# barathanaslan/whisper-ipa

Hardware: AMD Instinct MI355X
Metric: audio-seconds/sec transcribed (whisper-small, 30s clips) (higher is better)
Workload: dtype bf16

## Files before the change

### whisper_ipa_amd/csrc/attention.hip

```cpp
#include <cstring>

#include "attn_stream.h"
#include "wipa_common.h"

namespace {

struct AttnParams {
    const char* q;
    const char* k;
    const char* v;
    char* out;
    const int32_t* tk_dev;
    const int32_t* q_row_dev;
    float* lse;
    int64_t q_bs, q_rs, q_hs, k_bs, k_rs, k_hs, v_bs, v_rs, v_hs, o_bs, o_rs, o_hs;
    int Tq, Tk, causal, H;
};

template <bool RAGGED, bool GROUPED = false>
struct AttnArgs : AttnParams {};
template <>
struct AttnArgs<true> : AttnParams {
    const int32_t* k_start;
};
// ... 313 lines not shown
        Vec16<T> qv = *reinterpret_cast<const Vec16<T>*>(qp);
#pragma unroll
        for (int e = 0; e < EPL; ++e) qf[t][e] = qv.get(e);
    }
    int kvb = b;
    if constexpr (GROUPED) kvb = b / p.n_group;
    const T* Kb = reinterpret_cast<const T*>(p.k) + kvb * p.k_bs + h * p.k_hs + c * EPL;
    const T* Vb = reinterpret_cast<const T*>(p.v) + kvb * p.v_bs + h * p.v_hs + c * EPL;
    const int64_t k_rs = p.k_rs, v_rs = p.v_rs;
    float m[NQ], l[NQ], acc[NQ][EPL];
#pragma unroll
    for (int t = 0; t < NQ; ++t) {
        m[t] = NEG_BIG;
        l[t] = 0.f;
#pragma unroll
        for (int e = 0; e < EPL; ++e) acc[t][e] = 0.f;
    }
    constexpr int STEP = 4 * G * U;
    for (int t0 = wave * G * U; t0 < Tk; t0 += STEP) {
        Vec16<T> ka[U], va[U];
#pragma unroll
        for (int u = 0; u < U; ++u) {
            ka[u] = load_row_clamped(Kb, t0 + u * G + g, Tk - 1, k_rs);
            va[u] = load_row_clamped(Vb, t0 + u * G + g, Tk - 1, v_rs);
        }
#pragma unroll
        for (int t = 0; t < NQ; ++t) WIPA_STREAM_STEP(U, qf[t], ka, va, t0, m[t], l[t], acc[t]);
    }
#pragma unroll
    for (int t = 0; t < NQ; ++t) {
        WIPA_LANE_MERGE(LPK, 64, EPL, m[t], l[t], acc[t]);
        WIPA_WAVE_MERGE_STORE(s_acc[t], s_m[t], s_l[t], m[t], l[t], acc[t]);
    }
    __syncthreads();
    if (tid < 64 * NQ) {
        const int t = tid >> 6, dd = tid & 63;
        WIPA_WAVE_MERGE_OUT(s_acc[t], s_m[t], s_l[t], dd, reinterpret_cast<T*>(p.out)[b * p.o_bs + (int64_t)t * p.o_rs + h * p.o_hs + dd]);
    }
}

constexpr int FA_ROWB = 128;
constexpr int FA_TILE = 64 * FA_ROWB;
constexpr float LOG2E = 1.4426950408889634f;

#define WIPA_FLASH_SOFTMAX_TILE()                                                                  \
    do {                                                                                           \
        if (kt * 64 + 64 > T) {                                                                    \
            asm volatile("" ::: "memory");                                                         \
            _Pragma("unroll") for (int u = 0; u < 2; ++u)                                          \
                _Pragma("unroll") for (int i = 0; i < 16; ++i) {                                   \
                    const int key = kt * 64 + 32 * u + (i & 3) + 8 * (i >> 2) + 4 * hh;            \
                    if (key >= T) S[u][i] = NEG_BIG;                                               \
                }                                                                                  \
        }                                                                                          \
        float mx = NEG_BIG;                                                                        \
        _Pragma("unroll") for (int u = 0; u < 2; ++u)                                              \
            _Pragma("unroll") for (int i = 0; i < 16; ++i) mx = fmaxf(mx, S[u][i]);                \
        mx = fmaxf(mx, __shfl_xor(mx, 32, 64));                                                    \
        const float m_new = fmaxf(m, mx * LOG2E);                                                  \
        f32x2 psum2 = {0.f, 0.f};                                                                  \
        const f32x2 l2e = {LOG2E, LOG2E}, mneg = {-m_new, -m_new};                                 \
        _Pragma("unroll") for (int u = 0; u < 2; ++u)                                              \
            _Pragma("unroll") for (int i = 0; i < 16; i += 2) {                                    \
                const f32x2 x = __builtin_elementwise_fma(f32x2{S[u][i], S[u][i + 1]}, l2e, mneg); \
                const f32x2 pv = {__builtin_amdgcn_exp2f(x.x), __builtin_amdgcn_exp2f(x.y)};       \
                S[u][i] = pv.x;                                                                    \
                S[u][i + 1] = pv.y;                                                                \
                psum2 += pv;                                                                       \
            }                                                                                      \
        const float psum = psum2.x + psum2.y;                                                      \
        if (__any(m_new > m)) {                                                                    \
            const float alpha = __builtin_amdgcn_exp2f(m - m_new);                                 \
            l *= alpha;                                                                            \
            _Pragma("unroll") for (int i = 0; i < 16; ++i) {                                       \
                O[0][i] *= alpha;                                                                  \
                O[1][i] *= alpha;                                                                  \
            }                                                                                      \
            m = m_new;                                                                             \
        }                                                                                          \
        l += psum;                                                                                 \
    } while (0)
#define WIPA_FLASH_SOFTMAX_FINISH() l += __shfl_xor(l, 32, 64)

__global__ __launch_bounds__(512) void flash_enc_bf16_kernel(const __bf16* __restrict__ qk, int64_t ldqk,
                                                             const __bf16* __restrict__ vt, int64_t ldvt,
                                                             __bf16* __restrict__ out, int64_t ldo, int H, int T) {
    __shared__ __attribute__((aligned(16))) char smem[4 * FA_TILE];
    const int tid = threadIdx.x, lane = tid & 63, wave = tid >> 6;
    const int r = lane & 31, hh = lane >> 5;
    const int h = blockIdx.y, b = blockIdx.z;
    const int D = H * 64;
    const int nw = blockDim.x >> 6;
    const int q0 = blockIdx.x * (nw * 32) + wave * 32;
    const int nkt = (T + 63) / 64;

    bf16x8 qf[4];
    {
        const int qrow = min(q0 + r, T - 1);
        const __bf16* qp = qk + ((int64_t)b * T + qrow) * ldqk + h * 64 + 8 * hh;
#pragma unroll
        for (int s = 0; s < 4; ++s) qf[s] = *reinterpret_cast<const bf16x8*>(qp + 16 * s);
    }
    typedef __attribute__((address_space(3))) void* lds_t;
    const __bf16* kbase = qk + (int64_t)b * T * ldqk + D + h * 64;
    const __bf16* vbase = vt + ((int64_t)b * D + h * 64) * ldvt;
    const __amdgpu_buffer_rsrc_t rK = __builtin_amdgcn_make_buffer_rsrc((void*)kbase, 0, (int)(((int64_t)(T - 1) * ldqk + 64) * 2), 0x00020000);
    const __amdgpu_buffer_rsrc_t rV = __builtin_amdgcn_make_buffer_rsrc((void*)vbase, 0, (int)(((int64_t)63 * ldvt + ldvt) * 2), 0x00020000);
    const int wv = __builtin_amdgcn_readfirstlane(wave);
    const int ppw = 8 / nw;
    int offK[2], offV[2];
#pragma unroll
    for (int i = 0; i < 2; ++i) {
        const int row = 8 * (ppw * wv + i) + (lane >> 3);
        const int c = (lane & 7) ^ ((row >> 1) & 7);
        offK[i] = row * (int)ldqk * 2 + c * 16;
        offV[i] = row * (int)ldvt * 2 + c * 16;
    }
    auto stage = [&](int kt, int buf) {
        char* base = smem + buf * 2 * FA_TILE + (ppw * wv) * 1024;
        const int k0 = kt * 64;
#pragma unroll
        for (int i = 0; i < 2; ++i) {
            if (i < ppw) {
                __builtin_amdgcn_raw_ptr_buffer_load_lds(rK, (lds_t)(base + i * 1024), 16, offK[i], k0 * (int)ldqk * 2, 0, 0);
                __builtin_amdgcn_raw_ptr_buffer_load_lds(rV, (lds_t)(base + FA_TILE + i * 1024), 16, offV[i], k0 * 2, 0, 0);
            }
        }
    };

    f32x16 O[2];
#pragma unroll
    for (int i = 0; i < 16; ++i) O[0][i] = O[1][i] = 0.f;
    float m = NEG_BIG, l = 0.f;
    const int rsw = (r >> 1) & 7;

    stage(0, 0);
    asm volatile("s_waitcnt vmcnt(0)" ::: "memory");
    __syncthreads();
    for (int kt = 0; kt < nkt; ++kt) {
        if (kt + 1 < nkt) stage(kt + 1, (kt + 1) & 1);
        const char* kbuf = smem + (kt & 1) * 2 * FA_TILE;
        const char* vbuf = kbuf + FA_TILE;
        f32x16 S[2];
#pragma unroll
        for (int u = 0; u < 2; ++u) {
#pragma unroll
            for (int i = 0; i < 16; ++i) S[u][i] = 0.f;
            const char* krow = kbuf + (32 * u + r) * FA_ROWB;
#pragma unroll
            for (int s = 0; s < 4; ++s) {
                const bf16x8 kf = *reinterpret_cast<const bf16x8*>(krow + (((2 * s + hh) ^ rsw) << 4));
                S[u] = __builtin_amdgcn_mfma_f32_32x32x16_bf16(kf, qf[s], S[u], 0, 0, 0);
            }
        }
        WIPA_FLASH_SOFTMAX_TILE();
#pragma unroll
        for (int u = 0; u < 2; ++u)
#pragma unroll
            for (int sp = 0; sp < 2; ++sp) {
                bf16x8 pb;
#pragma unroll
                for (int j = 0; j < 8; ++j) pb[j] = (__bf16)S[u][8 * sp + j];
#pragma unroll
                for (int dt = 0; dt < 2; ++dt) {
                    const char* vrow = vbuf + (32 * dt + r) * FA_ROWB + 8 * hh;
                    const int c0 = 4 * u + 2 * sp;
                    const bf16x4 lo = *reinterpret_cast<const bf16x4*>(vrow + ((c0 ^ rsw) << 4));
                    const bf16x4 hi = *reinterpret_cast<const bf16x4*>(vrow + (((c0 + 1) ^ rsw) << 4));
                    const bf16x8 vf = {lo[0], lo[1], lo[2], lo[3], hi[0], hi[1], hi[2], hi[3]};
                    O[dt] = __builtin_amdgcn_mfma_f32_32x32x16_bf16(vf, pb, O[dt], 0, 0, 0);
                    asm volatile("" ::: "memory");
                }
            }
        asm volatile("s_waitcnt vmcnt(0)" ::: "memory");
        __syncthreads();
    }
    WIPA_FLASH_SOFTMAX_FINISH();
    const int qrow = q0 + r;
    if (qrow < T) {
        const float inv = 1.f / l;
        __bf16* op = out + ((int64_t)b * T + qrow) * ldo + h * 64 + 4 * hh;
#pragma unroll
        for (int dt = 0; dt < 2; ++dt)
#pragma unroll
            for (int g4 = 0; g4 < 4; ++g4) {
                bf16x4 o = {(__bf16)(O[dt][4 * g4] * inv), (__bf16)(O[dt][4 * g4 + 1] * inv),
                            (__bf16)(O[dt][4 * g4 + 2] * inv), (__bf16)(O[dt][4 * g4 + 3] * inv)};
                *reinterpret_cast<bf16x4*>(op + 32 * dt + 8 * g4) = o;
            }
    }
}

constexpr int FF_LD = 68;
constexpr int FF_TILE = 64 * FF_LD;

__device__ __forceinline__ void stage_k_parity(float* krow, int kseg, const f32x4 (&rk)[4]) {
    float* kt = krow + 8 * kseg;
    *reinterpret_cast<f32x4*>(kt) = f32x4{rk[0][0], rk[0][2], rk[1][0], rk[1][2]};
    *reinterpret_cast<f32x4*>(kt + 4) = f32x4{rk[2][0], rk[2][2], rk[3][0], rk[3][2]};
    *reinterpret_cast<f32x4*>(kt + 32) = f32x4{rk[0][1], rk[0][3], rk[1][1], rk[1][3]};
    *reinterpret_cast<f32x4*>(kt + 36) = f32x4{rk[2][1], rk[2][3], rk[3][1], rk[3][3]};
}
__device__ __forceinline__ void stage_k_plain(float* krow, int kseg, const f32x4 (&rk)[4]) {
    float* kt = krow + 16 * kseg;
#pragma unroll
    for (int c = 0; c < 4; ++c) *reinterpret_cast<f32x4*>(kt + 4 * c) = rk[c];
}

#define WIPA_FLASH_F32_INDICES()                                                                                 \
    __shared__ __attribute__((aligned(16))) float smem[4 * FF_TILE];     \
    const int tid = threadIdx.x, lane = tid & 63, wave = tid >> 6;                                               \
    const int r = lane & 31, hh = lane >> 5;                                                                     \
    const int h = blockIdx.y, b = blockIdx.z;                                                                    \
    const int q0 = blockIdx.x * 128 + wave * 32;                                                                 \
    const int nkt = (T + 63) / 64

#define WIPA_FLASH_F32_STAGING(STAGE_K)                                                                          \
    const int krow = tid >> 2, kseg = tid & 3;                                                                   \
    const int vkey = tid & 63, vseg = tid >> 6;                                                                  \
    const float* kg = k + (int64_t)b * T * ldk + h * 64 + 16 * kseg;                                             \
    const float* vg = v + (int64_t)b * T * ldv + h * 64 + 16 * vseg;                                             \
    f32x4 rk[4], rv[4];                                                                                          \
    auto gload = [&](int kt) {                                                                                   \
        const float* kp = kg + (int64_t)min(kt * 64 + krow, T - 1) * ldk;                                        \
        const float* vp = vg + (int64_t)min(kt * 64 + vkey, T - 1) * ldv;                                        \
        _Pragma("unroll") for (int c = 0; c < 4; ++c) {                                                          \
            rk[c] = *reinterpret_cast<const f32x4*>(kp + 4 * c);                                                 \
            rv[c] = *reinterpret_cast<const f32x4*>(vp + 4 * c);                                                 \
        }                                                                                                        \
    };                                                                                                           \
    auto swrite = [&](int buf) {                                                                                 \
        STAGE_K(smem + buf * 2 * FF_TILE + krow * FF_LD, kseg, rk);                                              \
        float* vt = smem + buf * 2 * FF_TILE + FF_TILE + (16 * vseg) * FF_LD + vkey;            \
        _Pragma("unroll") for (int c = 0; c < 4; ++c)                                                            \
            _Pragma("unroll") for (int e = 0; e < 4; ++e) vt[(4 * c + e) * FF_LD] = rv[c][e];                    \
    };                                                                                                           \
    f32x16 O[2];                                                                                                 \
    _Pragma("unroll") for (int i = 0; i < 16; ++i) O[0][i] = O[1][i] = 0.f;                                      \
    float m = NEG_BIG, l = 0.f;                                                        \
    gload(0);                                                                                                    \
    swrite(0);                                                                                                   \
    __syncthreads()

#define WIPA_FLASH_F32_TILE_BEGIN()                                                                              \
    if (kt + 1 < nkt) gload(kt + 1);                                                                             \
    const float* kbuf = smem + (kt & 1) * 2 * FF_TILE;                                                           \
    const float* vbuf = kbuf + FF_TILE;                                                                          \
    f32x16 S[2]
#define WIPA_FLASH_F32_TILE_END()                                                                                \
    if (kt + 1 < nkt) swrite((kt + 1) & 1);                                                                      \
    __syncthreads()

#define WIPA_FLASH_F32_TAIL()                                                                                    \
    WIPA_FLASH_SOFTMAX_FINISH();                                                                                 \
    const int qrow = q0 + r;                                                                                     \
    if (qrow < T) {                                                                                              \
        const float inv = 1.f / l;                                                                               \
        float* op = out + ((int64_t)b * T + qrow) * ldo + h * 64 + 4 * hh;                                       \
// ... 33 lines not shown
#pragma unroll
        for (int u = 0; u < 2; ++u)
#pragma unroll
            for (int dt = 0; dt < 2; ++dt) {
                const float* vr = vbuf + (32 * dt + r) * FF_LD + 32 * u + 4 * hh;
#pragma unroll
                for (int g = 0; g < 4; ++g) {
                    const f32x4 vf = *reinterpret_cast<const f32x4*>(vr + 8 * g);
#pragma unroll
                    for (int e = 0; e < 4; ++e)
                        O[dt] = __builtin_amdgcn_mfma_f32_32x32x2f32(vf[e], S[u][4 * g + e], O[dt], 0, 0, 0);
                }
            }
        WIPA_FLASH_F32_TILE_END();
    }
    WIPA_FLASH_F32_TAIL();
}

__global__ __launch_bounds__(256, 2) void flash_enc_f32s_kernel(const float* __restrict__ q, int64_t ldq,
                                                                const float* __restrict__ k, int64_t ldk,
                                                                const float* __restrict__ v, int64_t ldv,
                                                                float* __restrict__ out, int64_t ldo, int T) {
    WIPA_FLASH_F32_INDICES();
    bf16x8 qh[4], qm[4], ql[4];
    {
        const float* qp = q + ((int64_t)b * T + min(q0 + r, T - 1)) * ldq + h * 64 + 8 * hh;
#pragma unroll
        for (int s = 0; s < 4; ++s)
            split_bf16x3(*reinterpret_cast<const f32x4*>(qp + 16 * s), *reinterpret_cast<const f32x4*>(qp + 16 * s + 4), qh[s], qm[s], ql[s]);
    }
    WIPA_FLASH_F32_STAGING(stage_k_plain);
    for (int kt = 0; kt < nkt; ++kt) {
        WIPA_FLASH_F32_TILE_BEGIN();
#pragma unroll
        for (int u = 0; u < 2; ++u) {
#pragma unroll
            for (int i = 0; i < 16; ++i) S[u][i] = 0.f;
            const float* kr = kbuf + (32 * u + r) * FF_LD + 8 * hh;
#pragma unroll
            for (int s = 0; s < 4; ++s) {
                bf16x8 kh, km, kl;
                split_bf16x3(*reinterpret_cast<const f32x4*>(kr + 16 * s), *reinterpret_cast<const f32x4*>(kr + 16 * s + 4), kh, km, kl);
                S[u] = __builtin_amdgcn_mfma_f32_32x32x16_bf16(kl, qh[s], S[u], 0, 0, 0);
                S[u] = __builtin_amdgcn_mfma_f32_32x32x16_bf16(km, qm[s], S[u], 0, 0, 0);
                S[u] = __builtin_amdgcn_mfma_f32_32x32x16_bf16(kh, ql[s], S[u], 0, 0, 0);
                S[u] = __builtin_amdgcn_mfma_f32_32x32x16_bf16(km, qh[s], S[u], 0, 0, 0);
                S[u] = __builtin_amdgcn_mfma_f32_32x32x16_bf16(kh, qm[s], S[u], 0, 0, 0);
                S[u] = __builtin_amdgcn_mfma_f32_32x32x16_bf16(kh, qh[s], S[u], 0, 0, 0);
            }
        }
        WIPA_FLASH_SOFTMAX_TILE();
#pragma unroll
        for (int u = 0; u < 2; ++u)
#pragma unroll
            for (int sp = 0; sp < 2; ++sp) {
                bf16x8 ph, pl;
                split_bf16x2(f32x4{S[u][8 * sp], S[u][8 * sp + 1], S[u][8 * sp + 2], S[u][8 * sp + 3]},
                             f32x4{S[u][8 * sp + 4], S[u][8 * sp + 5], S[u][8 * sp + 6], S[u][8 * sp + 7]}, ph, pl);
#pragma unroll
                for (int dt = 0; dt < 2; ++dt) {
                    const float* vr = vbuf + (32 * dt + r) * FF_LD + 32 * u + 16 * sp + 4 * hh;
                    bf16x8 vh, vl;
                    split_bf16x2(*reinterpret_cast<const f32x4*>(vr), *reinterpret_cast<const f32x4*>(vr + 8), vh, vl);
                    O[dt] = __builtin_amdgcn_mfma_f32_32x32x16_bf16(vh, pl, O[dt], 0, 0, 0);
                    O[dt] = __builtin_amdgcn_mfma_f32_32x32x16_bf16(vl, ph, O[dt], 0, 0, 0);
                    O[dt] = __builtin_amdgcn_mfma_f32_32x32x16_bf16(vh, ph, O[dt], 0, 0, 0);
                }
            }
        WIPA_FLASH_F32_TILE_END();
    }
    WIPA_FLASH_F32_TAIL();
}

#undef WIPA_FLASH_F32_INDICES
#undef WIPA_FLASH_F32_STAGING
#undef WIPA_FLASH_F32_TILE_BEGIN
#undef WIPA_FLASH_F32_TILE_END
#undef WIPA_FLASH_F32_TAIL
#undef WIPA_FLASH_SOFTMAX_TILE
#undef WIPA_FLASH_SOFTMAX_FINISH

}

static bool attn_strides_aligned(const wipa_attn_desc* d) {
    const int64_t al = d->dtype == WIPA_BF16 ? 8 : 4;
    return d->q_rs % al == 0 && d->k_rs % al == 0 && d->v_rs % al == 0 && d->q_hs % al == 0 && d->k_hs % al == 0 && d->v_hs % al == 0 &&
           d->q_bs % al == 0 && d->k_bs % al == 0 && d->v_bs % al == 0;
}

static void fill_attn_params(const wipa_attn_desc* d, AttnParams& p) {
    p.q = (const char*)d->q;
    p.k = (const char*)d->k;
    p.v = (const char*)d->v;
    p.out = (char*)d->out;
    p.tk_dev = d->tk_dev;
    p.q_row_dev = d->q_row_dev;
    p.lse = d->lse;
    p.q_bs = d->q_bs; p.q_rs = d->q_rs; p.q_hs = d->q_hs;
    p.k_bs = d->k_bs; p.k_rs = d->k_rs; p.k_hs = d->k_hs;
    p.v_bs = d->v_bs; p.v_rs = d->v_rs; p.v_hs = d->v_hs;
    p.o_bs = d->o_bs; p.o_rs = d->o_rs; p.o_hs = d->o_hs;
    p.Tq = d->Tq;
    p.Tk = d->Tk;
    p.causal = d->causal;
    p.H = d->H;
}

extern "C" int wipa_attention(const wipa_attn_desc* d, wipa_stream_t stream) { return wipa_attention_as(d, d ? d->Tq : 0, stream); }

int wipa_attention_as(const wipa_attn_desc* d, int path_tq, wipa_stream_t stream) {
    WIPA_REQUIRE(d && d->q && d->k && d->v && d->out, "wipa_attention: null pointer");
    WIPA_REQUIRE(d->B > 0 && d->H > 0 && d->Tq > 0, "wipa_attention: bad shape");
    WIPA_REQUIRE(d->dtype == WIPA_F32 || d->dtype == WIPA_BF16, "wipa_attention: bad dtype %d", d->dtype);
    WIPA_REQUIRE(attn_strides_aligned(d), "wipa_attention: strides must keep 16-byte alignment");
    AttnArgs<false> p;
    fill_attn_params(d, p);
    dim3 grid((d->Tq + 15) / 16, d->H, d->B);
    static const bool valu = [] { const char* e = getenv("WIPA_ATTN_FWD"); return e && !strcmp(e, "valu"); }();
    if (d->dtype == WIPA_F32 && !valu && path_tq >= 16 && !d->tk_dev && !d->q_row_dev && d->o_rs % 4 == 0 && d->o_hs % 4 == 0 &&
        d->o_bs % 4 == 0) {
        hipLaunchKernelGGL(attn_fwd_f32_mfma_kernel, dim3((d->Tq + 63) / 64, d->H, d->B), dim3(256), 0, (hipStream_t)stream, p);
        WIPA_LAUNCH_CHECK();
        return WIPA_OK;
    }
    if (d->dtype == WIPA_F32)
        hipLaunchKernelGGL((attn_generic_kernel<float>), grid, dim3(256), 0, (hipStream_t)stream, p);
    else
        hipLaunchKernelGGL((attn_generic_kernel<__bf16>), grid, dim3(256), 0, (hipStream_t)stream, p);
    WIPA_LAUNCH_CHECK();
    return WIPA_OK;
}

extern "C" int wipa_attention_ragged(const wipa_attn_desc* d, const int32_t* starts_dev, wipa_stream_t stream) {
    WIPA_REQUIRE(d && d->q && d->k && d->v && d->out && starts_dev, "wipa_attention_ragged: null pointer (starts_dev is required)");
    WIPA_REQUIRE(d->B > 0 && d->H > 0 && d->Tq > 0, "wipa_attention_ragged: bad shape");
    WIPA_REQUIRE(d->dtype == WIPA_F32 || d->dtype == WIPA_BF16, "wipa_attention_ragged: bad dtype %d", d->dtype);
    WIPA_REQUIRE(attn_strides_aligned(d), "wipa_attention_ragged: strides must keep 16-byte alignment");
    WIPA_REQUIRE(d->causal && d->Tq == d->Tk && !d->tk_dev && !d->q_row_dev && !d->lse,
                 "wipa_attention_ragged: causal self-attention with Tq == Tk (Tq=%d Tk=%d), no device-side offsets, no lse", d->Tq, d->Tk);
    AttnArgs<true> p;
    fill_attn_params(d, p);
    p.k_start = starts_dev;
    dim3 grid((d->Tq + 15) / 16, d->H, d->B);
    if (d->dtype == WIPA_F32)
        hipLaunchKernelGGL((attn_generic_kernel<float, true>), grid, dim3(256), 0, (hipStream_t)stream, p);
    else
        hipLaunchKernelGGL((attn_generic_kernel<__bf16, true>), grid, dim3(256), 0, (hipStream_t)stream, p);
    WIPA_LAUNCH_CHECK();
    return WIPA_OK;
}

extern "C" int wipa_flash_attn_enc_bf16(const void* qk, int64_t ldqk, const void* vt, int64_t ldvt, void* out, int64_t ldo,
                                        int B, int H, int T, wipa_stream_t stream) {
    WIPA_REQUIRE(qk && vt && out, "wipa_flash_attn_enc_bf16: null pointer");
    WIPA_REQUIRE(ldqk % 8 == 0 && ldvt % 8 == 0 && ldo % 4 == 0, "wipa_flash_attn_enc_bf16: ld alignment");
    WIPA_REQUIRE(ldvt >= ((T + 63) / 64) * 64, "wipa_flash_attn_enc_bf16: ldvt=%lld must cover ceil64(T)", (long long)ldvt);
    WIPA_REQUIRE(B > 0 && H > 0 && T > 0, "wipa_flash_attn_enc_bf16: bad shape");
    static const int q128 = [] { const char* e = getenv("WIPA_FLASH_Q128"); return e ? atoi(e) : 0; }();
    const int nw = (T > 256 && !q128) ? 8 : 4;
    dim3 grid((T + nw * 32 - 1) / (nw * 32), H, B);
    hipLaunchKernelGGL(flash_enc_bf16_kernel, grid, dim3(nw * 64), 0, (hipStream_t)stream, (const __bf16*)qk, ldqk,
                       (const __bf16*)vt, ldvt, (__bf16*)out, ldo, H, T);
    WIPA_LAUNCH_CHECK();
    return WIPA_OK;
}

extern "C" int wipa_flash_attn_enc_f32(const float* q, int64_t ldq, const float* k, int64_t ldk, const float* v, int64_t ldv,
                                       float* out, int64_t ldo, int B, int H, int T, int f32_split, wipa_stream_t stream) {
    WIPA_REQUIRE(q && k && v && out, "wipa_flash_attn_enc_f32: null pointer");
    WIPA_REQUIRE(ldq % 4 == 0 && ldk % 4 == 0 && ldv % 4 == 0 && ldo % 4 == 0, "wipa_flash_attn_enc_f32: row strides must be multiples of 4");
    WIPA_REQUIRE(((uintptr_t)q % 16) == 0 && ((uintptr_t)k % 16) == 0 && ((uintptr_t)v % 16) == 0 && ((uintptr_t)out % 16) == 0,
                 "wipa_flash_attn_enc_f32: operands must be 16-byte aligned");
    WIPA_REQUIRE(B > 0 && H > 0 && T > 0, "wipa_flash_attn_enc_f32: bad shape");
    dim3 grid((T + 127) / 128, H, B);
    if (!f32_split)
        hipLaunchKernelGGL(flash_enc_f32_kernel, grid, dim3(256), 0, (hipStream_t)stream, q, ldq, k, ldk, v, ldv, out, ldo, T);
    else
        hipLaunchKernelGGL(flash_enc_f32s_kernel, grid, dim3(256), 0, (hipStream_t)stream, q, ldq, k, ldk, v, ldv, out, ldo, T);
    WIPA_LAUNCH_CHECK();
    return WIPA_OK;
}

extern "C" int wipa_decode_attn(const wipa_attn_desc* d, wipa_stream_t stream) {
    WIPA_REQUIRE(d && d->q && d->k && d->v && d->out, "wipa_decode_attn: null pointer");
    WIPA_REQUIRE(d->B > 0 && d->H > 0 && d->Tq == 1, "wipa_decode_attn: one query row per (b,h) (Tq=%d)", d->Tq);
    WIPA_REQUIRE(d->dtype == WIPA_F32 || d->dtype == WIPA_BF16, "wipa_decode_attn: bad dtype %d", d->dtype);
    WIPA_REQUIRE(attn_strides_aligned(d), "wipa_decode_attn: strides must keep 16-byte alignment");
    AttnArgs<false> p;
    fill_attn_params(d, p);
    const bool short_cache = d->Tk + (d->tk_dev ? 448 : 0) <= 512;
    static const int self_waves = [] { const char* e = getenv("WIPA_SELF_ATTN_WAVES"); return e ? atoi(e) : 4; }();
    if (short_cache && self_waves == 4) {
        dim3 grid(d->H, d->B);
        if (d->dtype == WIPA_F32)
            hipLaunchKernelGGL((decode_attn_kernel<float, 4, false>), grid, dim3(256), 0, (hipStream_t)stream, p);
        else
            hipLaunchKernelGGL((decode_attn_kernel<__bf16, 4, false>), grid, dim3(256), 0, (hipStream_t)stream, p);
    } else if (short_cache) {
        dim3 grid((d->H + 3) / 4, d->B);
        if (d->dtype == WIPA_F32)
            hipLaunchKernelGGL((decode_attn_kernel<float, 1>), grid, dim3(256), 0, (hipStream_t)stream, p);
        else
            hipLaunchKernelGGL((decode_attn_kernel<__bf16, 1>), grid, dim3(256), 0, (hipStream_t)stream, p);
    } else {
        dim3 grid(d->H, d->B);
        if (d->dtype == WIPA_F32)
            hipLaunchKernelGGL((decode_attn_kernel<float, 4>), grid, dim3(256), 0, (hipStream_t)stream, p);
        else
            hipLaunchKernelGGL((decode_attn_kernel<__bf16, 4>), grid, dim3(256), 0, (hipStream_t)stream, p);
    }
    WIPA_LAUNCH_CHECK();
    return WIPA_OK;
}

extern "C" int wipa_decode_attn_ragged(const wipa_attn_desc* d, const int32_t* starts_dev, wipa_stream_t stream) {
    WIPA_REQUIRE(d && d->q && d->k && d->v && d->out && starts_dev, "wipa_decode_attn_ragged: null pointer (starts_dev is required)");
    WIPA_REQUIRE(d->B > 0 && d->H > 0 && d->Tq == 1, "wipa_decode_attn_ragged: one query row per (b,h) (Tq=%d)", d->Tq);
    WIPA_REQUIRE(d->dtype == WIPA_F32 || d->dtype == WIPA_BF16, "wipa_decode_attn_ragged: bad dtype %d", d->dtype);
    WIPA_REQUIRE(attn_strides_aligned(d), "wipa_decode_attn_ragged: strides must keep 16-byte alignment");
    WIPA_REQUIRE(d->q_row_dev && d->tk_dev, "wipa_decode_attn_ragged: the query row and the key count come from the device (q_row_dev, tk_dev)");
    AttnArgs<true> p;
    fill_attn_params(d, p);
    p.k_start = starts_dev;
    dim3 grid(d->H, d->B);
    if (d->dtype == WIPA_F32)
        hipLaunchKernelGGL((decode_attn_kernel<float, 4, false, true>), grid, dim3(256), 0, (hipStream_t)stream, p);
    else
        hipLaunchKernelGGL((decode_attn_kernel<__bf16, 4, false, true>), grid, dim3(256), 0, (hipStream_t)stream, p);
    WIPA_LAUNCH_CHECK();
    return WIPA_OK;
}

static wipa_attn_desc cross_attn_desc(const void* q, const void* kv, void* out, int B, int H, int Tk, int n_q, int dtype) {
    wipa_attn_desc d;
    memset(&d, 0, sizeof(d));
    const size_t e = wipa_dtype_size(dtype);
    d.q = q; d.k = kv; d.v = (const char*)kv + (size_t)H * Tk * 64 * e; d.out = out;
    d.q_bs = (int64_t)n_q * H * 64; d.q_rs = (int64_t)H * 64; d.q_hs = 64;
    d.k_bs = (int64_t)2 * H * Tk * 64; d.k_rs = 64; d.k_hs = (int64_t)Tk * 64;
    d.v_bs = d.k_bs; d.v_rs = 64; d.v_hs = d.k_hs;
    d.o_bs = d.q_bs; d.o_rs = d.q_rs; d.o_hs = 64;
    d.B = B; d.H = H; d.Tq = n_q; d.Tk = Tk; d.causal = 0; d.dtype = dtype;
    return d;
}

// ... 72 lines not shown
```

### whisper_ipa_amd/csrc/gemm.hip

```cpp
#include <atomic>
#include <cstdlib>
#include <cstring>
#include <mutex>

#include <type_traits>

#include "wipa_common.h"

namespace {

struct GemmParams {
    int f32_split = 0;
    const char* A;
    const char* W;
    char* C;
    const float* bias;
    const char* residual;
    const float* pos;
    const int64_t* c_offset_dev;
    int64_t lda_b, ldw_b;
    int64_t ldc, ldpos;
    int64_t rg_stride, cg_stride, c_offset;
    int M, N, K;
    int rg_in, rg_valid, cg_in;
// ... 191 lines not shown
        asm volatile("s_waitcnt lgkmcnt(0)" ::: "memory");
#pragma unroll
        for (int pass = 0; pass < NPASS; ++pass) {
            const int row = pass * RPP + rrow;
            float v[EPC];
#pragma unroll
            for (int t = 0; t < NCH; ++t) {
                const f32x4 a = *reinterpret_cast<const f32x4*>(scratch + row * 256 + (((cch * NCH + t) ^ row) << 4));
#pragma unroll
                for (int e = 0; e < 4; ++e) v[4 * t + e] = a[e];
            }
            const EpiRow R = epi_row(p, m_base + 16 * j + row, coff_dev);
            if (!R.store || !col_ok) continue;
            const int64_t off = R.roff + coff;
#pragma unroll
            for (int e = 0; e < EPC; ++e) v[e] = (v[e] + bias[e] + R.bm) * sc;
            if constexpr (ACT) {
                if (p.act == 1) {
#pragma unroll
                    for (int e = 0; e < EPC; e += 2) {
                        const f32x2 g = gelu_erf2(f32x2{v[e], v[e + 1]});
                        v[e] = g.x;
                        v[e + 1] = g.y;
                    }
                }
            }
            if (p.pos) {
#pragma unroll
                for (int e = 0; e < EPC; ++e)
                    if (e < nvalid) v[e] += p.pos[(int64_t)R.gr * p.ldpos + n + e];
            }
            const bool full = nvalid == EPC;
            if (p.residual) {
                const OutT* rp = reinterpret_cast<const OutT*>(p.residual) + off;
                if (full) {
                    if constexpr (PREFETCH) {
#pragma unroll
                        for (int e = 0; e < EPC; ++e) v[e] += rcur[pass].get(e);
                    } else {
                        typedef decltype(rcur[pass].v) VT;
                        Vec16<OutT> rr;
                        rr.v = __builtin_nontemporal_load(reinterpret_cast<const VT*>(rp));
#pragma unroll
                        for (int e = 0; e < EPC; ++e) v[e] += rr.get(e);
                    }
                } else {
#pragma unroll
                    for (int e = 0; e < EPC; ++e)
                        if (e < nvalid) v[e] += to_f32<OutT>(rp[e]);
                }
            }
            if (!R.valid) {
#pragma unroll
                for (int e = 0; e < EPC; ++e) v[e] = 0.f;
            }
            OutT* cp = reinterpret_cast<OutT*>(p.C) + off;
            if (full) {
                if constexpr (sizeof(OutT) == 4) {
                    __builtin_nontemporal_store(f32x4{v[0], v[1], v[2], v[3]}, reinterpret_cast<f32x4*>(cp));
                } else {
                    __builtin_nontemporal_store(bf16x8{(__bf16)v[0], (__bf16)v[1], (__bf16)v[2], (__bf16)v[3],
                                                            (__bf16)v[4], (__bf16)v[5], (__bf16)v[6], (__bf16)v[7]}, reinterpret_cast<bf16x8*>(cp));
                }
            } else {
#pragma unroll
                for (int e = 0; e < EPC; ++e)
                    if (e < nvalid) cp[e] = from_f32<OutT>(v[e]);
            }
        }
        asm volatile("s_waitcnt lgkmcnt(0)" ::: "memory");
    }
}

constexpr int BM = 128, BN = 128, ROWB = 128;
constexpr int TILE_BYTES = BM * ROWB;
constexpr int GROUP_M = 8;


struct TileId {
    int m, n;
};
__device__ __forceinline__ TileId tile_id(const GemmParams& p) {
    const int nblocks = p.tiles_m * p.tiles_n;
    int id;
    {
        const int bid = blockIdx.x;
        const int q = nblocks >> 3, r = nblocks & 7;
        const int xcd = bid & 7, idx = bid >> 3;
        id = (xcd < r ? xcd * (q + 1) : r * (q + 1) + (xcd - r) * q) + idx;
    }
    const int group_size = GROUP_M * p.tiles_n;
    const int group = id / group_size;
    const int first_m = group * GROUP_M;
    const int gm = min(p.tiles_m - first_m, GROUP_M);
    const int in_group = id - group * group_size;
    return {first_m + in_group % gm, in_group / gm};
}

struct FragLane {
    int frow, fsw, fq;
};
__device__ __forceinline__ FragLane frag_lane(int lane) { return {lane & 15, (lane >> 1) & 7, lane >> 4}; }

#define WIPA_ZERO_ACC(NI, NJ) \
    _Pragma("unroll") for (int i = 0; i < (NI); ++i) _Pragma("unroll") for (int j = 0; j < (NJ); ++j) acc[i][j] = f32x4{0.f, 0.f, 0.f, 0.f}

#define WIPA_STORE_TILE_DIRECT(OutT, MT, m_base, n_base, coff_dev, vec)                                      \
    EpiCol cols[4];                                                                                          \
    _Pragma("unroll") for (int i = 0; i < 4; ++i) cols[i] = epi_col(p, (n_base) + 16 * i + 4 * fq);          \
    _Pragma("unroll") for (int j = 0; j < (MT); ++j) {                                                       \
        const EpiRow row = epi_row(p, (m_base) + 16 * j + frow, coff_dev);                                   \
        _Pragma("unroll") for (int i = 0; i < 4; ++i) epilogue4<OutT>(p, acc[i][j], row, cols[i], vec);      \
    }

#define WIPA_BIAS_GELU_MFMA(MT, n_base)                                                                      \
    _Pragma("unroll") for (int i = 0; i < 4; ++i) {                                                          \
        const int n = (n_base) + 16 * i + 4 * fq;                                                            \
        float b4[4];                                                                                         \
        _Pragma("unroll") for (int e = 0; e < 4; ++e) b4[e] = (p.bias && n + e < p.N) ? p.bias[n + e] : 0.f; \
        _Pragma("unroll") for (int j = 0; j < (MT); ++j) {                                                   \
            const f32x2 g0 = gelu_erf2(f32x2{acc[i][j][0] + b4[0], acc[i][j][1] + b4[1]});                   \
            const f32x2 g1 = gelu_erf2(f32x2{acc[i][j][2] + b4[2], acc[i][j][3] + b4[3]});                   \
            acc[i][j] = f32x4{g0.x, g0.y, g1.x, g1.y};                                                       \
            __builtin_amdgcn_sched_barrier(0);  \
        }                                                                                                    \
    }                                                                                                        \
    p.bias = nullptr;

enum { GELU_IN_EPILOGUE, GELU_NONE, GELU_FIRST };
#define WIPA_STORE_TILE(OutT, MT, GELU, STAGED_ONLY, m_base, n_base)                                         \
    [[maybe_unused]] const bool vec = p.vec_ok != 0;                                                         \
    int64_t coff_dev = p.c_offset;                                                                           \
    if (p.c_offset_dev) coff_dev += *p.c_offset_dev;                                                         \
    if ((STAGED_ONLY) || p.stage_ok) {                                                                       \
        if constexpr ((GELU) == GELU_FIRST) {                                                                \
            WIPA_BIAS_GELU_MFMA(MT, n_base)                                                                  \
        }                                                                                                    \
        epilogue_staged<OutT, MT, 0, MT, (GELU) == GELU_IN_EPILOGUE, (GELU) != GELU_FIRST>(p, acc, smem + wave * 4096, m_base, n_base, \
                                                                                           coff_dev, lane); \
        return;                                                                                              \
    }                                                                                                        \
    if constexpr (!(STAGED_ONLY)) {                                                                          \
        WIPA_STORE_TILE_DIRECT(OutT, MT, m_base, n_base, coff_dev, vec)                                      \
    }

template <int BM_, int BN_, bool ZIP_>
struct TileGeom {
    static constexpr int BM = BM_, BN = BN_;
    static constexpr int WN = BN / 64;
    static constexpr int MT = BM * WN / 128;
    static constexpr int W_PIECES = BN / 64, A_PIECES = BM / 64;
    static constexpr int W_TILE = BN * ROWB;
    static constexpr int STAGE = W_TILE + BM * ROWB;
    static constexpr int SMEM = 2 * STAGE;
    static constexpr bool ZIP = ZIP_;
    static_assert(W_PIECES <= A_PIECES && (!ZIP || W_PIECES == A_PIECES), "stager loop bounds");
};

typedef __attribute__((address_space(3))) void* lds_ptr_t;

__device__ __forceinline__ __amdgpu_buffer_rsrc_t tile_rsrc(const char* base, int row0, int64_t ld_b) {
    return __builtin_amdgcn_make_buffer_rsrc((void*)(base + (int64_t)row0 * ld_b), 0, 0x7fffffff, 0x00020000);
}
__device__ __forceinline__ int dma_offset(int row, int lane, int row0, int rows, int64_t ld_b) {
    return (min(row0 + row, rows - 1) - row0) * (int)ld_b + (((lane & 7) ^ ((row >> 1) & 7)) << 4);
}
#define WIPA_TILE_STAGER(G)                                                                                                               \
    const __amdgpu_buffer_rsrc_t rW = tile_rsrc(p.W, n0, p.ldw_b);                                                                        \
    const __amdgpu_buffer_rsrc_t rA = tile_rsrc(p.A, m0, p.lda_b);                                                                        \
    int oW[G::W_PIECES], oA[G::A_PIECES];                                                                                                 \
    _Pragma("unroll") for (int i = 0; i < G::A_PIECES; ++i) {                                                                             \
        const int row = 64 * i + 8 * wave + (lane >> 3);                                                                                  \
        const int c = (lane & 7) ^ ((row >> 1) & 7);                                                                                      \
// ... 1470 lines not shown
```

### whisper_ipa_amd/csrc/wipa_common.h

```cpp
#pragma once
#include <hip/hip_runtime.h>
#include <stdint.h>
#include <stdio.h>

#include "wipa.h"

typedef __attribute__((ext_vector_type(8))) __bf16 bf16x8;
typedef __attribute__((ext_vector_type(4))) __bf16 bf16x4;
typedef __attribute__((ext_vector_type(4))) float f32x4;
typedef __attribute__((ext_vector_type(16))) float f32x16;

#define WIPA_WAVE 64

void wipa_set_error(const char* fmt, ...);
int wipa_decode_fused_init();
int wipa_gemm_init();
int wipa_cross_absorbed_loop_variant();
int wipa_attention_as(const wipa_attn_desc* d, int path_tq, wipa_stream_t stream);
int wipa_step_tail(const float* logits, int64_t ldl, int B, int V, const float* mask_first, const float* mask_always, int32_t* tokens,
                   int64_t ld_tok, int32_t* pos_dev, int64_t* posd_dev, int32_t* done_counter, int n_init, int eot, const wipa_decode_rules* rules,
                   const void* sample, const int32_t* starts_dev, float* sum_logprobs, int32_t* not_done, const void* tok_emb, int emb_dtype,
                   const float* emb_scale, const float* pos_emb, int n_ctx, float* x, const float* ln_w, const float* ln_b, void* y, int y_dtype,
                   int D, float eps, wipa_stream_t stream);
int wipa_step_tail_continuous(const float* logits, int64_t ldl, int B, int V, const float* mask_first, const float* mask_always, int32_t* tokens,
                              int64_t ld_tok, int32_t* pos_dev, int64_t* posd_dev, int32_t* done_counter, int n_init, int eot, const void* sample,
                              const int32_t* starts_dev, float* sum_logprobs, int32_t* not_done, const void* tok_emb, int emb_dtype,
                              const float* emb_scale, const float* pos_emb, int n_ctx, float* x, const float* ln_w, const float* ln_b, void* y,
                              int y_dtype, int D, float eps, wipa_stream_t stream);
int wipa_step_tail_continuous_rules(const float* logits, int64_t ldl, int B, int V, const float* mask_first, const float* mask_always,
                                    int32_t* tokens, int64_t ld_tok, int32_t* pos_dev, int64_t* posd_dev, int32_t* done_counter, int n_init, int eot,
                                    const wipa_decode_rules* rules, const void* sample, const int32_t* starts_dev, float* no_speech_dev,
                                    int no_speech_token, float* sum_logprobs, int32_t* not_done, const void* tok_emb, int emb_dtype,
                                    const float* emb_scale, const float* pos_emb, int n_ctx, float* x, const float* ln_w, const float* ln_b, void* y,
                                    int y_dtype, int D, float eps, wipa_stream_t stream);
int wipa_step_tail_continuous_rows(const float* logits, int64_t ldl, int B, int V, const float* mask_first, const float* mask_always,
                                   int32_t* tokens, int64_t ld_tok, int32_t* pos_dev, int64_t* posd_dev, int32_t* done_counter, int n_init, int eot,
                                   const wipa_decode_rules* rules, const void* sample_rows, const int32_t* starts_dev, float* no_speech_dev,
                                   int no_speech_token, float* sum_logprobs, int32_t* not_done, const void* tok_emb, int emb_dtype,
                                   const float* emb_scale, const float* pos_emb, int n_ctx, float* x, const float* ln_w, const float* ln_b, void* y,
                                   int y_dtype, int D, float eps, wipa_stream_t stream);

#define WIPA_CHECK_HIP(expr)                                                        \
    do {                                                                            \
        hipError_t _e = (expr);                                                     \
        if (_e != hipSuccess) {                                                     \
            wipa_set_error("%s:%d %s -> %s", __FILE__, __LINE__, #expr, hipGetErrorString(_e)); \
            return WIPA_ERR_HIP;                                                    \
        }                                                                           \
    } while (0)

#define WIPA_REQUIRE(cond, ...)                \
    do {                                       \
        if (!(cond)) {                         \
            wipa_set_error(__VA_ARGS__);       \
            return WIPA_ERR_ARG;               \
        }                                      \
    } while (0)

#define WIPA_LAUNCH_CHECK()                                                          \
    do {                                                                             \
        hipError_t _e = hipGetLastError();                                           \
        if (_e != hipSuccess) {                                                      \
            wipa_set_error("%s:%d launch -> %s", __FILE__, __LINE__, hipGetErrorString(_e)); \
            return WIPA_ERR_HIP;                                                     \
        }                                                                            \
    } while (0)

static inline size_t wipa_dtype_size(int dt) { return dt == WIPA_BF16 ? 2 : 4; }

#ifdef __HIPCC__
__device__ __forceinline__ float wipa_bf16_to_f32(unsigned short h) {
    return __uint_as_float(((unsigned int)h) << 16);
}

template <typename T>
__device__ __forceinline__ float to_f32(T v);
template <>
__device__ __forceinline__ float to_f32<float>(float v) { return v; }
template <>
__device__ __forceinline__ float to_f32<__bf16>(__bf16 v) { return (float)v; }

template <typename T>
__device__ __forceinline__ T from_f32(float v);
template <>
__device__ __forceinline__ float from_f32<float>(float v) { return v; }
template <>
__device__ __forceinline__ __bf16 from_f32<__bf16>(float v) { return (__bf16)v; }

template <typename T>
struct Vec16;
template <>
struct Vec16<float> {
    static constexpr int EPL = 4;
    f32x4 v;
    __device__ __forceinline__ float get(int i) const { return v[i]; }
};
template <>
struct Vec16<__bf16> {
    static constexpr int EPL = 8;
    bf16x8 v;
    __device__ __forceinline__ float get(int i) const { return (float)v[i]; }
};

__device__ __forceinline__ float wave_reduce_sum(float v) {
#pragma unroll
    for (int o = 32; o > 0; o >>= 1) v += __shfl_xor(v, o, 64);
    return v;
}
__device__ __forceinline__ float wave_reduce_max(float v) {
#pragma unroll
    for (int o = 32; o > 0; o >>= 1) v = fmaxf(v, __shfl_xor(v, o, 64));
    return v;
}

template <typename T>
struct Mma;
template <>
struct Mma<__bf16> {
    typedef bf16x8 Frag;
    static __device__ __forceinline__ void run(const Frag& w, const Frag& x, f32x4& acc) {
        acc = __builtin_amdgcn_mfma_f32_16x16x32_bf16(w, x, acc, 0, 0, 0);
    }
};
template <>
struct Mma<float> {
    typedef f32x4 Frag;
    static __device__ __forceinline__ void run(const Frag& w, const Frag& x, f32x4& acc) {
#pragma unroll
        for (int e = 0; e < 4; ++e) acc = __builtin_amdgcn_mfma_f32_16x16x4f32(w[e], x[e], acc, 0, 0, 0);
    }
};

__device__ __forceinline__ float erf_fast(float x) {
    const float ax = fabsf(x);
    const float t = __builtin_amdgcn_rcpf(fmaf(0.3275911f, ax, 1.0f));
    float p = fmaf(1.061405429f, t, -1.453152027f);
    p = fmaf(p, t, 1.421413741f);
    p = fmaf(p, t, -0.284496736f);
    p = fmaf(p, t, 0.254829592f);
    const float e = __builtin_amdgcn_exp2f(-1.4426950408889634f * ax * ax);
    const float y = fmaf(-p * t, e, 1.0f);
    return copysignf(y, x);
}
__device__ __forceinline__ float gelu_erf(float x) { return 0.5f * x * (1.0f + erf_fast(x * 0.70710678118654752440f)); }

typedef float f32x2 __attribute__((ext_vector_type(2)));
__device__ __forceinline__ f32x2 gelu_erf2(f32x2 x) {
    const f32x2 ax = __builtin_elementwise_abs(x);
    const f32x2 d = __builtin_elementwise_fma(f32x2{0.2316418882f, 0.2316418882f}, ax, f32x2{1.f, 1.f});
    const f32x2 t = {__builtin_amdgcn_rcpf(d.x), __builtin_amdgcn_rcpf(d.y)};
    f32x2 p = __builtin_elementwise_fma(f32x2{0.5307027145f, 0.5307027145f}, t, f32x2{-0.7265760135f, -0.7265760135f});
    p = __builtin_elementwise_fma(p, t, f32x2{0.7107068705f, 0.7107068705f});
    p = __builtin_elementwise_fma(p, t, f32x2{-0.142248368f, -0.142248368f});
    p = __builtin_elementwise_fma(p, t, f32x2{0.127414796f, 0.127414796f});
    p = p * t;
    const f32x2 s = x * 0.8493218003f;
    const f32x2 s2 = s * s;
    const f32x2 e = {__builtin_amdgcn_exp2f(-s2.x), __builtin_amdgcn_exp2f(-s2.y)};
    return __builtin_elementwise_fma(-ax, p * e, __builtin_elementwise_max(x, f32x2{0.f, 0.f}));
}
__device__ __forceinline__ void split_bf16x2(const f32x4& a, const f32x4& b, bf16x8& hi, bf16x8& lo) {
    const float x[8] = {a[0], a[1], a[2], a[3], b[0], b[1], b[2], b[3]};
#pragma unroll
    for (int e = 0; e < 8; ++e) {
        const __bf16 h = (__bf16)x[e];
        hi[e] = h;
        lo[e] = (__bf16)(x[e] - (float)h);
    }
}


__device__ __forceinline__ void split_bf16x3(const f32x4& a, const f32x4& b, bf16x8& hi, bf16x8& mid, bf16x8& lo) {
    const float x[8] = {a[0], a[1], a[2], a[3], b[0], b[1], b[2], b[3]};
#pragma unroll
    for (int e = 0; e < 8; ++e) {
        const __bf16 h = (__bf16)x[e];
        const float r1 = x[e] - (float)h;
        const __bf16 m = (__bf16)r1;
        hi[e] = h;
        mid[e] = m;
        lo[e] = (__bf16)(r1 - (float)m);
    }
}

#endif
```

Measured before the change: 27530.

## Add triple-buffered K/V ring and XCD-contiguous block mapping to encoder flash attention

Templates the encoder flash-attention kernel on a variant mask. It can prefetch K/V two tiles ahead through a three-slot LDS ring, using partial vmcnt waits and raw s_barrier in place of a full drain each tile. It can also remap the flattened grid so consecutive query tiles of the same batch-head land on the same XCD, improving L2 reuse of K/V. Both are on by default via an env var, and the XCD remap helper is shared with the GEMM tile mapper. The cost is 50% more LDS per block, which may lower occupancy, plus more complex wait-count logic.

New measurement: 27750, median of 6. About the same (+0.8%).

```diff
diff --git a/whisper_ipa_amd/csrc/attention.hip b/whisper_ipa_amd/csrc/attention.hip
--- a/whisper_ipa_amd/csrc/attention.hip
+++ b/whisper_ipa_amd/csrc/attention.hip
@@ -419,16 +419,30 @@
     } while (0)
 #define WIPA_FLASH_SOFTMAX_FINISH() l += __shfl_xor(l, 32, 64)
 
+constexpr int FA_CHAIN_RING = 2;
+constexpr int FA_CHAIN_XCD = 4;
+
+template <int CHAIN>
 __global__ __launch_bounds__(512) void flash_enc_bf16_kernel(const __bf16* __restrict__ qk, int64_t ldqk,
                                                              const __bf16* __restrict__ vt, int64_t ldvt,
                                                              __bf16* __restrict__ out, int64_t ldo, int H, int T) {
-    __shared__ __attribute__((aligned(16))) char smem[4 * FA_TILE];
+    constexpr bool RING = (CHAIN & FA_CHAIN_RING) != 0, XCD = (CHAIN & FA_CHAIN_XCD) != 0;
+    constexpr int NSLOT = RING ? 3 : 2;
+    __shared__ __attribute__((aligned(16))) char smem[NSLOT * 2 * FA_TILE];
     const int tid = threadIdx.x, lane = tid & 63, wave = tid >> 6;
     const int r = lane & 31, hh = lane >> 5;
-    const int h = blockIdx.y, b = blockIdx.z;
+    const int nw = blockDim.x >> 6;
+    int qt = blockIdx.x, h = blockIdx.y, b = blockIdx.z;
+    if constexpr (XCD) {
+        const int nqt = (T + nw * 32 - 1) / (nw * 32);
+        const int id = xcd_contiguous_id(blockIdx.x, gridDim.x);
+        const int bh = id / nqt;
+        qt = id - bh * nqt;
+        b = bh / H;
+        h = bh - b * H;
+    }
     const int D = H * 64;
-    const int nw = blockDim.x >> 6;
-    const int q0 = blockIdx.x * (nw * 32) + wave * 32;
+    const int q0 = qt * (nw * 32) + wave * 32;
     const int nkt = (T + 63) / 64;
 
     bf16x8 qf[4];
@@ -471,12 +485,7 @@
     float m = NEG_BIG, l = 0.f;
     const int rsw = (r >> 1) & 7;
 
-    stage(0, 0);
-    asm volatile("s_waitcnt vmcnt(0)" ::: "memory");
-    __syncthreads();
-    for (int kt = 0; kt < nkt; ++kt) {
-        if (kt + 1 < nkt) stage(kt + 1, (kt + 1) & 1);
-        const char* kbuf = smem + (kt & 1) * 2 * FA_TILE;
+    auto tile = [&](int kt, const char* kbuf) __attribute__((always_inline)) {
         const char* vbuf = kbuf + FA_TILE;
         f32x16 S[2];
 #pragma unroll
@@ -509,8 +518,41 @@
                     asm volatile("" ::: "memory");
                 }
             }
+    };
+
+    if constexpr (!RING) {
+        stage(0, 0);
         asm volatile("s_waitcnt vmcnt(0)" ::: "memory");
         __syncthreads();
+        for (int kt = 0; kt < nkt; ++kt) {
+            if (kt + 1 < nkt) stage(kt + 1, (kt + 1) & 1);
+            tile(kt, smem + (kt & 1) * 2 * FA_TILE);
+            asm volatile("s_waitcnt vmcnt(0)" ::: "memory");
+            __syncthreads();
+        }
+    } else {
+        auto step = [&](int kt, int cur, int ahead) __attribute__((always_inline)) {
+            const bool more = kt + 2 < nkt;
+            if (more) stage(kt + 2, ahead);
+            tile(kt, smem + cur * 2 * FA_TILE);
+            if (!more) asm volatile("s_waitcnt vmcnt(0) lgkmcnt(0)" ::: "memory");
+            else if (ppw == 1) asm volatile("s_waitcnt vmcnt(2) lgkmcnt(0)" ::: "memory");
+            else asm volatile("s_waitcnt vmcnt(4) lgkmcnt(0)" ::: "memory");
+            __builtin_amdgcn_s_barrier();
+            asm volatile("" ::: "memory");
+        };
+        stage(0, 0);
+        if (nkt > 1) stage(1, 1);
+        asm volatile("s_waitcnt vmcnt(0)" ::: "memory");
+        __syncthreads();
+        for (int kt = 0;;) {
+            step(kt, 0, 2);
+            if (++kt == nkt) break;
+            step(kt, 1, 0);
+            if (++kt == nkt) break;
+            step(kt, 2, 1);
+            if (++kt == nkt) break;
+        }
     }
     WIPA_FLASH_SOFTMAX_FINISH();
     const int qrow = q0 + r;
@@ -710,6 +752,12 @@
 
 }
 
+static int wipa_flash_chain_variant() {
+    const char* e = getenv("WIPA_FLASH_CHAIN");
+    const int v = e ? atoi(e) : 7;
+    return ((v >= 0 && v <= 7) ? v : 7) & (FA_CHAIN_RING | FA_CHAIN_XCD);
+}
+
 static bool attn_strides_aligned(const wipa_attn_desc* d) {
     const int64_t al = d->dtype == WIPA_BF16 ? 8 : 4;
     return d->q_rs % al == 0 && d->k_rs % al == 0 && d->v_rs % al == 0 && d->q_hs % al == 0 && d->k_hs % al == 0 && d->v_hs % al == 0 &&
@@ -786,9 +834,21 @@
     WIPA_REQUIRE(B > 0 && H > 0 && T > 0, "wipa_flash_attn_enc_bf16: bad shape");
     static const int q128 = [] { const char* e = getenv("WIPA_FLASH_Q128"); return e ? atoi(e) : 0; }();
     const int nw = (T > 256 && !q128) ? 8 : 4;
-    dim3 grid((T + nw * 32 - 1) / (nw * 32), H, B);
-    hipLaunchKernelGGL(flash_enc_bf16_kernel, grid, dim3(nw * 64), 0, (hipStream_t)stream, (const __bf16*)qk, ldqk,
-                       (const __bf16*)vt, ldvt, (__bf16*)out, ldo, H, T);
+    const int nqt = (T + nw * 32 - 1) / (nw * 32);
+    WIPA_REQUIRE((int64_t)nqt * H * B <= INT32_MAX, "wipa_flash_attn_enc_bf16: too many workgroups");
+    switch (wipa_flash_chain_variant()) {
+#define WIPA_FLASH_CASE(C)                                                                                                       \
+    case C:                                                                                                                      \
+        hipLaunchKernelGGL(flash_enc_bf16_kernel<C>, ((C) & FA_CHAIN_XCD) ? dim3(nqt * H * B) : dim3(nqt, H, B), dim3(nw * 64), 0, \
+                           (hipStream_t)stream, (const __bf16*)qk, ldqk, (const __bf16*)vt, ldvt, (__bf16*)out, ldo, H, T);      \
+        break
+        WIPA_FLASH_CASE(0);
+        WIPA_FLASH_CASE(FA_CHAIN_RING);
+        WIPA_FLASH_CASE(FA_CHAIN_XCD);
+        default:
+        WIPA_FLASH_CASE(FA_CHAIN_RING | FA_CHAIN_XCD);
+#undef WIPA_FLASH_CASE
+    }
     WIPA_LAUNCH_CHECK();
     return WIPA_OK;
 }
diff --git a/whisper_ipa_amd/csrc/gemm.hip b/whisper_ipa_amd/csrc/gemm.hip
--- a/whisper_ipa_amd/csrc/gemm.hip
+++ b/whisper_ipa_amd/csrc/gemm.hip
@@ -297,13 +297,7 @@
 };
 __device__ __forceinline__ TileId tile_id(const GemmParams& p) {
     const int nblocks = p.tiles_m * p.tiles_n;
-    int id;
-    {
-        const int bid = blockIdx.x;
-        const int q = nblocks >> 3, r = nblocks & 7;
-        const int xcd = bid & 7, idx = bid >> 3;
-        id = (xcd < r ? xcd * (q + 1) : r * (q + 1) + (xcd - r) * q) + idx;
-    }
+    const int id = xcd_contiguous_id(blockIdx.x, nblocks);
     const int group_size = GROUP_M * p.tiles_n;
     const int group = id / group_size;
     const int first_m = group * GROUP_M;
diff --git a/whisper_ipa_amd/csrc/wipa_common.h b/whisper_ipa_amd/csrc/wipa_common.h
--- a/whisper_ipa_amd/csrc/wipa_common.h
+++ b/whisper_ipa_amd/csrc/wipa_common.h
@@ -102,6 +102,12 @@
     __device__ __forceinline__ float get(int i) const { return (float)v[i]; }
 };
 
+__device__ __forceinline__ int xcd_contiguous_id(int bid, int n) {
+    const int q = n >> 3, r = n & 7;
+    const int xcd = bid & 7, idx = bid >> 3;
+    return (xcd < r ? xcd * (q + 1) : r * (q + 1) + (xcd - r) * q) + idx;
+}
+
 __device__ __forceinline__ float wave_reduce_sum(float v) {
 #pragma unroll
     for (int o = 32; o > 0; o >>= 1) v += __shfl_xor(v, o, 64);
```
